# barathanaslan/whisper-ipa

Measured on AMD Instinct MI355X. Metric: audio-seconds/sec transcribed (whisper-small, 30s clips), higher is better.
Workload: dtype bf16

## Files before the change

### include/wipa.h

```cpp
#ifndef WIPA_H
#define WIPA_H
#include <stddef.h>
#include <stdint.h>
#ifdef __cplusplus
extern "C" {
#endif

typedef void* wipa_stream_t;

enum { WIPA_F32 = 0, WIPA_BF16 = 1, WIPA_FP8_E4M3 = 2  };
enum { WIPA_OK = 0, WIPA_ERR_ARG = -1, WIPA_ERR_HIP = -2, WIPA_ERR_STATE = -3 };

#define WIPA_N_SAMPLES 480000
#define WIPA_N_FRAMES 3000
#define WIPA_N_FFT 400
#define WIPA_HOP 160
#define WIPA_HEAD_DIM 64

int wipa_version(void);
const char* wipa_last_error(void);

int wipa_stream_create(wipa_stream_t* out);
int wipa_stream_create_cu_limited(int n_cus, wipa_stream_t* out);
int wipa_stream_destroy(wipa_stream_t s);
// ... 86 lines not shown
int wipa_embed_tokens(const int32_t* tokens, int64_t ld_tok, int B, int T, int t_start, const int32_t* pos_dev,
                      const void* tok_emb, int emb_dtype, const float* emb_scale, const float* pos_emb, float* x, int D,
                      wipa_stream_t s);

typedef struct wipa_attn_desc {
    const void* q;
    const void* k;
    const void* v;
    void* out;
    const int32_t* tk_dev;
    const int32_t* q_row_dev;
    float* lse;
    int64_t q_bs, q_rs, q_hs;
    int64_t k_bs, k_rs, k_hs;
    int64_t v_bs, v_rs, v_hs;
    int64_t o_bs, o_rs, o_hs;
    int32_t B, H, Tq, Tk;
    int32_t causal, dtype;
} wipa_attn_desc;
int wipa_attention(const wipa_attn_desc* d, wipa_stream_t s);

int wipa_flash_attn_enc_bf16(const void* qk, int64_t ldqk, const void* vt, int64_t ldvt, void* out, int64_t ldo,
                             int B, int H, int T, wipa_stream_t s);
int wipa_flash_attn_enc_f32(const float* q, int64_t ldq, const float* k, int64_t ldk, const float* v, int64_t ldv, float* out,
                            int64_t ldo, int B, int H, int T, int f32_split, wipa_stream_t s);

int wipa_decode_attn(const wipa_attn_desc* d, wipa_stream_t s);
int wipa_decode_cross_attn(const void* q, const void* kv, void* out, int B, int H, int Tk, int dtype,
                           wipa_stream_t s);
int wipa_decode_cross_attn_multi(const void* q, const void* kv, void* out, int B, int H, int Tk, int n_q, int dtype,
                                 wipa_stream_t s);

typedef struct wipa_self_block_desc {
    const float* x;
    const float* ln_w;
    const float* ln_b;
    const void* wqkv;
    const float* bqkv;
    const void* wo;
    void* kcache;
    void* vcache;
    const int32_t* pos;
    float* slabs;
    int64_t kv_batch_stride, slab_stride;
    int32_t B, d, H, dtype;
    float eps, qk_scale;
// ... 68 lines not shown
typedef struct wipa_model_cfg {
    int32_t n_mels, n_audio_ctx, n_audio_state, n_audio_head, n_audio_layer;
    int32_t n_vocab, n_text_ctx, n_text_state, n_text_head, n_text_layer;
    int32_t dtype;
    int32_t f32_split;
    int32_t dec_w_dtype;
    int32_t weights_generation;
    int32_t enc_act_fp8;
    int32_t dec_cross_absorbed;
    int32_t dec_cross_splits;
} wipa_model_cfg;

#define WIPA_ENC_GLOBAL 7
#define WIPA_ENC_PER_LAYER 14
#define WIPA_ENC_FP8_PER_LAYER 8
#define WIPA_DEC_GLOBAL 4
#define WIPA_DEC_PER_LAYER 20
#define WIPA_DEC_FP8_PER_LAYER 6
#define WIPA_DEC_ABSORBED_PER_LAYER 1

size_t wipa_encoder_workspace_bytes(const wipa_model_cfg* cfg, int B);
int wipa_encoder_forward(const wipa_model_cfg* cfg, const void* const* weights, const void* mel_padded, void* out,
                         void* workspace, size_t workspace_bytes, int B, wipa_stream_t s);

#define WIPA_PROFILE_CLASSES 4
int wipa_profile_begin(wipa_stream_t s);
int wipa_profile_end(float* ms_by_class, int* launches_by_class);

typedef struct wipa_dec_layout {
    int64_t total_bytes;
    int64_t tokens;
    int64_t ld_tok;
    int64_t pos;
    int64_t not_done;
    int64_t sum_logprobs;
    int64_t logits;
    int64_t ld_logits;
    int64_t cross_kv;
    int64_t self_kv;
    int64_t scratch;
} wipa_dec_layout;
int wipa_decoder_layout(const wipa_model_cfg* cfg, int B, wipa_dec_layout* out);
int wipa_decoder_set_audio(const wipa_model_cfg* cfg, const void* const* weights, const void* features, void* state,
                           size_t state_bytes, int B, wipa_stream_t s);
int wipa_decoder_begin(const wipa_model_cfg* cfg, void* state, size_t state_bytes, int B, const int32_t* initial_tokens_host,
                       int n_init, wipa_stream_t s);
// ... 42 lines not shown
```

### whisper_ipa_amd/_lib.py

```python
from __future__ import annotations

import ctypes as C
import os
import threading

_HERE = os.path.dirname(os.path.abspath(__file__))
LIB_PATH = os.path.join(_HERE, "libwipa.so")

WIPA_F32, WIPA_BF16, WIPA_FP8_E4M3 = 0, 1, 2
GREEDY_PARTS = 2048
RESAMPLE_TILE = 512
ENC_GLOBAL, ENC_PER_LAYER = 7, 14
DEC_GLOBAL, DEC_PER_LAYER, DEC_FP8_PER_LAYER = 4, 20, 6
GEMM_DISPATCH = ("tile128", "tile256", "tile384", "tile384n", "tile256p", "skinny", "skinny_fp8", "skinny_ln", "kmajor", "split_k",
                 "tile_fp8", "tile_fp8_384")
ENC_FP8_PER_LAYER = 8
DEC_ABSORBED_PER_LAYER = 1

c_void_p, c_int, c_int64, c_size_t, c_float = C.c_void_p, C.c_int, C.c_int64, C.c_size_t, C.c_float


class GemmDesc(C.Structure):
    _fields_ = [
        ("A", c_void_p), ("W", c_void_p), ("C", c_void_p), ("bias", c_void_p), ("residual", c_void_p),
# ... 72 lines not shown
    "wipa_stream_create_cu_limited": (c_int, [c_int, C.POINTER(c_void_p)]),
    "wipa_stream_destroy": (c_int, [c_void_p]),
    "wipa_resample_pad": (c_int, [c_void_p, c_size_t, c_void_p, _P(PcmClipDesc), c_int, c_void_p, c_size_t, c_void_p, c_void_p]),
    "wipa_logmel_tables_bytes": (c_size_t, [c_int]),
    "wipa_logmel_init": (c_int, [c_void_p, c_int, c_void_p]),
    "wipa_logmel_workspace_bytes": (c_size_t, [c_int, c_int]),
    "wipa_logmel": (c_int, [c_void_p, c_int, c_int, c_void_p, c_void_p, c_int, c_void_p, c_size_t, c_void_p]),
    "wipa_mel_pad_cast": (c_int, [c_void_p, c_int, c_int, c_void_p, c_int, c_void_p]),
    "wipa_gemm": (c_int, [_P(GemmDesc), c_void_p]),
    "wipa_gemm_dispatch_counts": (c_int, [_P(c_int64), c_int, c_int]),
    "wipa_layernorm": (c_int, [c_void_p, c_int, c_int64, c_void_p, c_int, c_int64, c_void_p, c_void_p, c_int, c_int,
                               c_float, c_void_p]),
    "wipa_layernorm_fp8": (c_int, [c_void_p, c_int64, c_void_p, c_int64, c_void_p, c_void_p, c_void_p, c_int, c_int, c_float, c_void_p]),
    "wipa_rowquant_fp8": (c_int, [c_void_p, c_int, c_int64, c_void_p, c_int64, c_void_p, c_int, c_int, c_void_p]),
    "wipa_add_slabs_layernorm": (c_int, [c_void_p, c_int64, c_void_p, c_int, c_int64, c_void_p, c_int, c_int64, c_void_p,
                                         c_void_p, c_int, c_int, c_float, c_void_p]),
    "wipa_embed_tokens": (c_int, [c_void_p, c_int64, c_int, c_int, c_int, c_void_p, c_void_p, c_int, c_void_p, c_void_p, c_void_p,
                                  c_int, c_void_p]),
    "wipa_attention": (c_int, [_P(AttnDesc), c_void_p]),
    "wipa_flash_attn_enc_f32": (c_int, [c_void_p, c_int64, c_void_p, c_int64, c_void_p, c_int64, c_void_p, c_int64, c_int, c_int,
                                       c_int, c_int, c_void_p]),
    "wipa_flash_attn_enc_bf16": (c_int, [c_void_p, c_int64, c_void_p, c_int64, c_void_p, c_int64, c_int, c_int, c_int,
                                         c_void_p]),
    "wipa_decode_attn": (c_int, [_P(AttnDesc), c_void_p]),
    "wipa_decode_cross_attn": (c_int, [c_void_p, c_void_p, c_void_p, c_int, c_int, c_int, c_int, c_void_p]),
    "wipa_decode_self_block": (c_int, [_P(SelfBlockDesc), c_void_p]),
    "wipa_decode_cross_block": (c_int, [_P(CrossBlockDesc), c_void_p]),
    "wipa_cross_absorbed_splits": (c_int, [c_int, c_int]),
    "wipa_cross_absorbed_resident_groups_for": (c_int, [c_int, c_int, c_int, c_int, c_int64]),
    "wipa_cross_absorbed_resident_groups": (c_int, [c_int, c_int, c_int, c_int]),
    "wipa_cross_absorbed_scratch_bytes": (c_size_t, [c_int, c_int, c_int]),
    "wipa_cross_absorbed_init": (c_int, [c_int]),
    "wipa_cross_absorbed_attention": (c_int, [c_void_p, c_int64, c_void_p, c_void_p, c_void_p, c_void_p, c_void_p, c_int64, c_void_p, c_size_t,
                                              c_int, c_int, c_int, c_int, c_float, c_int, c_void_p]),
    "wipa_cross_absorbed_stream": (c_int, [c_void_p, c_void_p, c_size_t, c_int, c_int, c_int, c_int, c_int, c_void_p]),
    "wipa_decode_cross_absorbed_block": (c_int, [_P(CrossBlockDesc), c_void_p, c_void_p, c_void_p, c_void_p, c_size_t, c_void_p]),
    "wipa_decode_cross_absorbed_block_out": (c_int, [_P(CrossBlockDesc), c_void_p, c_void_p, c_void_p, c_void_p, c_void_p, c_void_p, c_int64,
                                                     c_void_p, c_size_t, c_void_p]),
    "wipa_greedy_step": (c_int, [c_void_p, c_int64, c_int, c_int, c_void_p, c_void_p, c_void_p, c_int64, c_void_p, c_int,
                                 c_int, c_void_p, c_void_p, c_void_p]),
    "wipa_add_i32": (c_int, [c_void_p, C.c_int32, c_void_p]),
    "wipa_greedy_step_embed": (c_int, [c_void_p, c_int64, c_int, c_int, c_void_p, c_void_p, c_void_p, c_int64, c_void_p, c_void_p, c_void_p,
                                       c_int, c_int, c_void_p, c_void_p, c_void_p, c_int, c_void_p, c_void_p, c_int, c_void_p, c_void_p,
                                       c_void_p, c_void_p, c_int, c_int, c_float, c_void_p]),
    "wipa_logits_greedy_supported": (c_int, [c_int, c_int, c_int, c_int]),
    "wipa_logits_greedy_partials_bytes": (c_size_t, [c_int]),
    "wipa_logits_greedy": (c_int, [c_void_p, c_int64, c_void_p, c_int64, c_void_p, c_int64, c_int, c_int, c_int, c_void_p, c_void_p, c_void_p,
                                   c_int, c_void_p, c_size_t, c_void_p]),
    "wipa_greedy_step_embed_partials": (c_int, [c_void_p, c_int, c_int, c_void_p, c_int64, c_void_p, c_void_p, c_void_p, c_int, c_int, c_void_p,
                                                c_void_p, c_void_p, c_int, c_void_p, c_void_p, c_int, c_void_p, c_void_p, c_void_p, c_void_p,
                                                c_int, c_int, c_float, c_void_p]),
    "wipa_embed_layernorm": (c_int, [c_void_p, c_int64, c_int, c_void_p, c_void_p, c_int, c_void_p, c_void_p, c_int, c_void_p, c_void_p,
                                     c_void_p, c_void_p, c_int, c_int, c_float, c_void_p]),
    "wipa_bpe_create": (c_void_p, [c_void_p, c_void_p, c_void_p, c_int]),
    "wipa_bpe_free": (None, [c_void_p]),
    "wipa_bpe_encode_piece": (c_int, [c_void_p, C.c_char_p, c_int, c_void_p, c_int]),
    "wipa_bpe_decode": (c_int, [c_void_p, c_void_p, c_int, c_void_p, c_int]),
    "wipa_build_token_batch": (c_int, [c_void_p, c_void_p, c_int, c_void_p, c_int, C.c_int32, c_void_p, c_int64]),
    "wipa_profile_begin": (c_int, [c_void_p]),
    "wipa_profile_end": (c_int, [_P(c_float), _P(c_int)]),
    "wipa_encoder_workspace_bytes": (c_size_t, [_P(ModelCfg), c_int]),
    "wipa_encoder_forward": (c_int, [_P(ModelCfg), _P(c_void_p), c_void_p, c_void_p, c_void_p, c_size_t, c_int, c_void_p]),
    "wipa_decoder_layout": (c_int, [_P(ModelCfg), c_int, _P(DecLayout)]),
    "wipa_decoder_set_audio": (c_int, [_P(ModelCfg), _P(c_void_p), c_void_p, c_void_p, c_size_t, c_int, c_void_p]),
    "wipa_decoder_begin": (c_int, [_P(ModelCfg), c_void_p, c_size_t, c_int, _P(C.c_int32), c_int, c_void_p]),
    "wipa_decoder_run": (c_int, [_P(ModelCfg), _P(c_void_p), c_void_p, c_size_t, c_int, c_int, c_int, c_void_p, c_void_p, c_int,
                                 c_int, c_void_p]),
    "wipa_decoder_prefill": (c_int, [_P(ModelCfg), _P(c_void_p), c_void_p, c_size_t, c_int, c_int, c_int, c_void_p, c_void_p, c_int,
                                     c_void_p]),
    "wipa_decode_cross_attn_multi": (c_int, [c_void_p, c_void_p, c_void_p, c_int, c_int, c_int, c_int, c_int, c_void_p]),
    "wipa_decoder_release": (c_int, [c_void_p]),
    "wipa_decoder_logits_workspace_bytes": (c_size_t, [_P(ModelCfg), c_int, c_int]),
    "wipa_decoder_logits": (c_int, [_P(ModelCfg), _P(c_void_p), c_void_p, c_void_p, c_void_p, c_int64, c_void_p, c_size_t,
                                    c_int, c_int, c_void_p]),
    "wipa_masked_ce": (c_int, [c_void_p, c_int64, c_void_p, c_int64, c_int, c_int, c_int, c_int, c_void_p, c_void_p,
                               c_void_p]),
    "wipa_transpose": (c_int, [c_void_p, c_int64, c_void_p, c_int64, c_int, c_int, c_int, c_int, c_void_p]),
    "wipa_sum_slabs": (c_int, [c_void_p, c_int, c_int64, c_void_p, c_int64, c_int, c_void_p]),
    "wipa_sum_slabs_ex": (c_int, [c_void_p, c_int, c_int64, c_void_p, c_int64, c_void_p, c_float, c_void_p]),
    "wipa_colsum": (c_int, [c_void_p, c_int64, c_int, c_int, c_void_p, c_int, c_void_p, c_int64, c_void_p]),
    "wipa_layernorm_bwd": (c_int, [c_void_p, c_void_p, c_void_p, c_void_p, c_int, c_void_p, c_void_p, c_void_p, c_int64, c_int, c_int,
                                   c_float, c_void_p]),
    "wipa_gelu": (c_int, [c_void_p, c_void_p, c_int64, c_void_p]),
    "wipa_gelu_bwd": (c_int, [c_void_p, c_void_p, c_void_p, c_int64, c_void_p]),
    "wipa_masked_ce_bwd": (c_int, [c_void_p, c_int64, c_void_p, c_int64, c_int, c_int, c_int, c_void_p, c_void_p, c_void_p]),
# ... 40 lines not shown
```

### whisper_ipa_amd/csrc/attention.hip

```cpp
#include <cstring>

#include "attn_stream.h"
#include "wipa_common.h"

namespace {

struct AttnParams {
    const char* q;
    const char* k;
    const char* v;
    char* out;
    const int32_t* tk_dev;
    const int32_t* q_row_dev;
    float* lse;
    int64_t q_bs, q_rs, q_hs, k_bs, k_rs, k_hs, v_bs, v_rs, v_hs, o_bs, o_rs, o_hs;
    int Tq, Tk, causal, H;
};

constexpr int GA_LD = 68;

template <typename T>
__global__ __launch_bounds__(256) void attn_generic_kernel(AttnParams p) {
    __shared__ __attribute__((aligned(16))) float Ks[64 * GA_LD];
    __shared__ __attribute__((aligned(16))) float Vs[64 * GA_LD];
// ... 343 lines not shown
        const f32x2 l2e = {LOG2E, LOG2E}, mneg = {-m_new, -m_new};                                 \
        _Pragma("unroll") for (int u = 0; u < 2; ++u)                                              \
            _Pragma("unroll") for (int i = 0; i < 16; i += 2) {                                    \
                const f32x2 x = __builtin_elementwise_fma(f32x2{S[u][i], S[u][i + 1]}, l2e, mneg); \
                const f32x2 pv = {__builtin_amdgcn_exp2f(x.x), __builtin_amdgcn_exp2f(x.y)};       \
                S[u][i] = pv.x;                                                                    \
                S[u][i + 1] = pv.y;                                                                \
                psum2 += pv;                                                                       \
            }                                                                                      \
        const float psum = psum2.x + psum2.y;                                                      \
        if (__any(m_new > m)) {                                                                    \
            const float alpha = __builtin_amdgcn_exp2f(m - m_new);                                 \
            l *= alpha;                                                                            \
            _Pragma("unroll") for (int i = 0; i < 16; ++i) {                                       \
                O[0][i] *= alpha;                                                                  \
                O[1][i] *= alpha;                                                                  \
            }                                                                                      \
            m = m_new;                                                                             \
        }                                                                                          \
        l += psum;                                                                                 \
    } while (0)
#define WIPA_FLASH_SOFTMAX_FINISH() l += __shfl_xor(l, 32, 64)

__global__ __launch_bounds__(512) void flash_enc_bf16_kernel(const __bf16* __restrict__ qk, int64_t ldqk,
                                                             const __bf16* __restrict__ vt, int64_t ldvt,
                                                             __bf16* __restrict__ out, int64_t ldo, int H, int T) {
    __shared__ __attribute__((aligned(16))) char smem[4 * FA_TILE];
    const int tid = threadIdx.x, lane = tid & 63, wave = tid >> 6;
    const int r = lane & 31, hh = lane >> 5;
    const int h = blockIdx.y, b = blockIdx.z;
    const int D = H * 64;
    const int nw = blockDim.x >> 6;
    const int q0 = blockIdx.x * (nw * 32) + wave * 32;
    const int nkt = (T + 63) / 64;

    bf16x8 qf[4];
    {
        const int qrow = min(q0 + r, T - 1);
        const __bf16* qp = qk + ((int64_t)b * T + qrow) * ldqk + h * 64 + 8 * hh;
#pragma unroll
        for (int s = 0; s < 4; ++s) qf[s] = *reinterpret_cast<const bf16x8*>(qp + 16 * s);
    }
    typedef __attribute__((address_space(3))) void* lds_t;
    const __bf16* kbase = qk + (int64_t)b * T * ldqk + D + h * 64;
    const __bf16* vbase = vt + ((int64_t)b * D + h * 64) * ldvt;
    const __amdgpu_buffer_rsrc_t rK = __builtin_amdgcn_make_buffer_rsrc((void*)kbase, 0, (int)(((int64_t)(T - 1) * ldqk + 64) * 2), 0x00020000);
    const __amdgpu_buffer_rsrc_t rV = __builtin_amdgcn_make_buffer_rsrc((void*)vbase, 0, (int)(((int64_t)63 * ldvt + ldvt) * 2), 0x00020000);
    const int wv = __builtin_amdgcn_readfirstlane(wave);
    const int ppw = 8 / nw;
    int offK[2], offV[2];
#pragma unroll
    for (int i = 0; i < 2; ++i) {
        const int row = 8 * (ppw * wv + i) + (lane >> 3);
        const int c = (lane & 7) ^ ((row >> 1) & 7);
        offK[i] = row * (int)ldqk * 2 + c * 16;
        offV[i] = row * (int)ldvt * 2 + c * 16;
    }
    auto stage = [&](int kt, int buf) {
        char* base = smem + buf * 2 * FA_TILE + (ppw * wv) * 1024;
        const int k0 = kt * 64;
#pragma unroll
        for (int i = 0; i < 2; ++i) {
            if (i < ppw) {
                __builtin_amdgcn_raw_ptr_buffer_load_lds(rK, (lds_t)(base + i * 1024), 16, offK[i], k0 * (int)ldqk * 2, 0, 0);
                __builtin_amdgcn_raw_ptr_buffer_load_lds(rV, (lds_t)(base + FA_TILE + i * 1024), 16, offV[i], k0 * 2, 0, 0);
            }
        }
    };

    f32x16 O[2];
#pragma unroll
    for (int i = 0; i < 16; ++i) O[0][i] = O[1][i] = 0.f;
    float m = NEG_BIG, l = 0.f;
    const int rsw = (r >> 1) & 7;

    stage(0, 0);
    asm volatile("s_waitcnt vmcnt(0)" ::: "memory");
    __syncthreads();
    for (int kt = 0; kt < nkt; ++kt) {
        if (kt + 1 < nkt) stage(kt + 1, (kt + 1) & 1);
        const char* kbuf = smem + (kt & 1) * 2 * FA_TILE;
        const char* vbuf = kbuf + FA_TILE;
        f32x16 S[2];
#pragma unroll
        for (int u = 0; u < 2; ++u) {
#pragma unroll
            for (int i = 0; i < 16; ++i) S[u][i] = 0.f;
            const char* krow = kbuf + (32 * u + r) * FA_ROWB;
#pragma unroll
            for (int s = 0; s < 4; ++s) {
                const bf16x8 kf = *reinterpret_cast<const bf16x8*>(krow + (((2 * s + hh) ^ rsw) << 4));
                S[u] = __builtin_amdgcn_mfma_f32_32x32x16_bf16(kf, qf[s], S[u], 0, 0, 0);
            }
        }
        WIPA_FLASH_SOFTMAX_TILE();
#pragma unroll
        for (int u = 0; u < 2; ++u)
#pragma unroll
            for (int sp = 0; sp < 2; ++sp) {
                bf16x8 pb;
#pragma unroll
                for (int j = 0; j < 8; ++j) pb[j] = (__bf16)S[u][8 * sp + j];
#pragma unroll
                for (int dt = 0; dt < 2; ++dt) {
                    const char* vrow = vbuf + (32 * dt + r) * FA_ROWB + 8 * hh;
                    const int c0 = 4 * u + 2 * sp;
                    const bf16x4 lo = *reinterpret_cast<const bf16x4*>(vrow + ((c0 ^ rsw) << 4));
                    const bf16x4 hi = *reinterpret_cast<const bf16x4*>(vrow + (((c0 + 1) ^ rsw) << 4));
                    const bf16x8 vf = {lo[0], lo[1], lo[2], lo[3], hi[0], hi[1], hi[2], hi[3]};
                    O[dt] = __builtin_amdgcn_mfma_f32_32x32x16_bf16(vf, pb, O[dt], 0, 0, 0);
                    asm volatile("" ::: "memory");
                }
            }
        asm volatile("s_waitcnt vmcnt(0)" ::: "memory");
        __syncthreads();
    }
// ... 172 lines not shown
                             f32x4{S[u][8 * sp + 4], S[u][8 * sp + 5], S[u][8 * sp + 6], S[u][8 * sp + 7]}, ph, pl);
#pragma unroll
                for (int dt = 0; dt < 2; ++dt) {
                    const float* vr = vbuf + (32 * dt + r) * FF_LD + 32 * u + 16 * sp + 4 * hh;
                    bf16x8 vh, vl;
                    split_bf16x2(*reinterpret_cast<const f32x4*>(vr), *reinterpret_cast<const f32x4*>(vr + 8), vh, vl);
                    O[dt] = __builtin_amdgcn_mfma_f32_32x32x16_bf16(vh, pl, O[dt], 0, 0, 0);
                    O[dt] = __builtin_amdgcn_mfma_f32_32x32x16_bf16(vl, ph, O[dt], 0, 0, 0);
                    O[dt] = __builtin_amdgcn_mfma_f32_32x32x16_bf16(vh, ph, O[dt], 0, 0, 0);
                }
            }
        WIPA_FLASH_F32_TILE_END();
    }
    WIPA_FLASH_F32_TAIL();
}

#undef WIPA_FLASH_F32_INDICES
#undef WIPA_FLASH_F32_STAGING
#undef WIPA_FLASH_F32_TILE_BEGIN
#undef WIPA_FLASH_F32_TILE_END
#undef WIPA_FLASH_F32_TAIL
#undef WIPA_FLASH_SOFTMAX_TILE
#undef WIPA_FLASH_SOFTMAX_FINISH

}

static bool attn_strides_aligned(const wipa_attn_desc* d) {
    const int64_t al = d->dtype == WIPA_BF16 ? 8 : 4;
    return d->q_rs % al == 0 && d->k_rs % al == 0 && d->v_rs % al == 0 && d->q_hs % al == 0 && d->k_hs % al == 0 && d->v_hs % al == 0 &&
           d->q_bs % al == 0 && d->k_bs % al == 0 && d->v_bs % al == 0;
}

static void fill_attn_params(const wipa_attn_desc* d, AttnParams& p) {
    p.q = (const char*)d->q;
    p.k = (const char*)d->k;
    p.v = (const char*)d->v;
    p.out = (char*)d->out;
    p.tk_dev = d->tk_dev;
    p.q_row_dev = d->q_row_dev;
    p.lse = d->lse;
    p.q_bs = d->q_bs; p.q_rs = d->q_rs; p.q_hs = d->q_hs;
    p.k_bs = d->k_bs; p.k_rs = d->k_rs; p.k_hs = d->k_hs;
    p.v_bs = d->v_bs; p.v_rs = d->v_rs; p.v_hs = d->v_hs;
    p.o_bs = d->o_bs; p.o_rs = d->o_rs; p.o_hs = d->o_hs;
    p.Tq = d->Tq;
    p.Tk = d->Tk;
// ... 13 lines not shown
    if (d->dtype == WIPA_F32 && !valu && d->Tq >= 16 && !d->tk_dev && !d->q_row_dev && d->o_rs % 4 == 0 && d->o_hs % 4 == 0 &&
        d->o_bs % 4 == 0) {
        hipLaunchKernelGGL(attn_fwd_f32_mfma_kernel, dim3((d->Tq + 63) / 64, d->H, d->B), dim3(256), 0, (hipStream_t)stream, p);
        WIPA_LAUNCH_CHECK();
        return WIPA_OK;
    }
    if (d->dtype == WIPA_F32)
        hipLaunchKernelGGL((attn_generic_kernel<float>), grid, dim3(256), 0, (hipStream_t)stream, p);
    else
        hipLaunchKernelGGL((attn_generic_kernel<__bf16>), grid, dim3(256), 0, (hipStream_t)stream, p);
    WIPA_LAUNCH_CHECK();
    return WIPA_OK;
}

extern "C" int wipa_flash_attn_enc_bf16(const void* qk, int64_t ldqk, const void* vt, int64_t ldvt, void* out, int64_t ldo,
                                        int B, int H, int T, wipa_stream_t stream) {
    WIPA_REQUIRE(qk && vt && out, "wipa_flash_attn_enc_bf16: null pointer");
    WIPA_REQUIRE(ldqk % 8 == 0 && ldvt % 8 == 0 && ldo % 4 == 0, "wipa_flash_attn_enc_bf16: ld alignment");
    WIPA_REQUIRE(ldvt >= ((T + 63) / 64) * 64, "wipa_flash_attn_enc_bf16: ldvt=%lld must cover ceil64(T)", (long long)ldvt);
    WIPA_REQUIRE(B > 0 && H > 0 && T > 0, "wipa_flash_attn_enc_bf16: bad shape");
    static const int q128 = [] { const char* e = getenv("WIPA_FLASH_Q128"); return e ? atoi(e) : 0; }();
    const int nw = (T > 256 && !q128) ? 8 : 4;
    dim3 grid((T + nw * 32 - 1) / (nw * 32), H, B);
    hipLaunchKernelGGL(flash_enc_bf16_kernel, grid, dim3(nw * 64), 0, (hipStream_t)stream, (const __bf16*)qk, ldqk,
                       (const __bf16*)vt, ldvt, (__bf16*)out, ldo, H, T);
    WIPA_LAUNCH_CHECK();
    return WIPA_OK;
}

extern "C" int wipa_flash_attn_enc_f32(const float* q, int64_t ldq, const float* k, int64_t ldk, const float* v, int64_t ldv,
                                       float* out, int64_t ldo, int B, int H, int T, int f32_split, wipa_stream_t stream) {
    WIPA_REQUIRE(q && k && v && out, "wipa_flash_attn_enc_f32: null pointer");
    WIPA_REQUIRE(ldq % 4 == 0 && ldk % 4 == 0 && ldv % 4 == 0 && ldo % 4 == 0, "wipa_flash_attn_enc_f32: row strides must be multiples of 4");
    WIPA_REQUIRE(((uintptr_t)q % 16) == 0 && ((uintptr_t)k % 16) == 0 && ((uintptr_t)v % 16) == 0 && ((uintptr_t)out % 16) == 0,
                 "wipa_flash_attn_enc_f32: operands must be 16-byte aligned");
    WIPA_REQUIRE(B > 0 && H > 0 && T > 0, "wipa_flash_attn_enc_f32: bad shape");
    dim3 grid((T + 127) / 128, H, B);
    if (!f32_split)
        hipLaunchKernelGGL(flash_enc_f32_kernel, grid, dim3(256), 0, (hipStream_t)stream, q, ldq, k, ldk, v, ldv, out, ldo, T);
    else
        hipLaunchKernelGGL(flash_enc_f32s_kernel, grid, dim3(256), 0, (hipStream_t)stream, q, ldq, k, ldk, v, ldv, out, ldo, T);
    WIPA_LAUNCH_CHECK();
    return WIPA_OK;
}

extern "C" int wipa_decode_attn(const wipa_attn_desc* d, wipa_stream_t stream) {
    WIPA_REQUIRE(d && d->q && d->k && d->v && d->out, "wipa_decode_attn: null pointer");
    WIPA_REQUIRE(d->B > 0 && d->H > 0 && d->Tq == 1, "wipa_decode_attn: one query row per (b,h) (Tq=%d)", d->Tq);
// ... 74 lines not shown
```

### whisper_ipa_amd/csrc/runtime.hip

```cpp
#include <algorithm>
#include <cstdarg>
#include <cstdlib>
#include <cstring>
#include <strings.h>
#include <map>
#include <mutex>
#include <tuple>
#include <vector>

#include "wipa_common.h"

static thread_local char g_err[512] = "";
void wipa_set_error(const char* fmt, ...) {
    va_list ap;
    va_start(ap, fmt);
    vsnprintf(g_err, sizeof(g_err), fmt, ap);
    va_end(ap);
}
extern "C" const char* wipa_last_error(void) { return g_err; }
extern "C" int wipa_version(void) { return 100; }

extern "C" int wipa_stream_create_cu_limited(int n_cus, wipa_stream_t* out) {
    int dev = 0, total = 0;
    WIPA_CHECK_HIP(hipGetDevice(&dev));
// ... 142 lines not shown
    g.bias = bias; g.act = act; g.residual = residual;
    g.a_scale = a_scale; g.w_scale = w_scale;
    return wipa_gemm(&g, s);
}

struct EncWs {
    size_t c1, x, ln, qk, v, ao, h, total;
};
EncWs enc_ws(const wipa_model_cfg* c, int B) {
    const size_t e = wipa_dtype_size(c->dtype), d = c->n_audio_state, M = (size_t)B * c->n_audio_ctx;
    EncWs w;
    size_t o = 0;
    w.c1 = o; o += align256(((size_t)B * ROWS_IN + 4) * d * e);
    w.x = o;  o += align256(M * d * 4);
    w.ln = o; o += align256(M * d * e);
    w.qk = o; o += align256(M * 2 * d * e);
    w.v = o;  o += align256(c->dtype == WIPA_BF16 ? (size_t)B * d * T_ENC_PAD * e + 256 : M * d * e);
    w.ao = o; o += align256(M * d * e);
    w.h = o;  o += align256(M * 4 * d * e);
    w.total = o;
    return w;
}

}

extern "C" size_t wipa_encoder_workspace_bytes(const wipa_model_cfg* cfg, int B) {
    if (!cfg || B <= 0) return 0;
    return enc_ws(cfg, B).total;
}

extern "C" int wipa_encoder_forward(const wipa_model_cfg* cfg, const void* const* w, const void* mel_padded, void* out,
                                    void* workspace, size_t workspace_bytes, int B, wipa_stream_t stream) {
    RT_CALL(cfg_check(cfg));
    SplitScope split_scope(cfg);
    WIPA_REQUIRE(w && mel_padded && out && workspace && B > 0, "wipa_encoder_forward: null pointer / bad batch");
    const EncWs L = enc_ws(cfg, B);
    WIPA_REQUIRE(workspace_bytes >= L.total, "wipa_encoder_forward: workspace too small (%zu < %zu)", workspace_bytes, L.total);
    hipStream_t s = (hipStream_t)stream;
    const int dt = cfg->dtype;
    const size_t e = wipa_dtype_size(dt);
    const int d = cfg->n_audio_state, H = cfg->n_audio_head, T = cfg->n_audio_ctx, M = B * T;
    char* ws = (char*)workspace;
    void* c1 = ws + L.c1;
    float* x = (float*)(ws + L.x);
    void* ln = ws + L.ln;
    void* qk = ws + L.qk;
    void* vb = ws + L.v;
    void* ao = ws + L.ao;
    void* hb = ws + L.h;
    const int K1 = round_up(3 * cfg->n_mels, k_multiple(dt));

    WIPA_CHECK_HIP(hipMemsetAsync(c1, 0, (size_t)d * e, s));
    {
        wipa_gemm_desc g;
        memset(&g, 0, sizeof(g));
        g.rg_in = ROWS_IN; g.rg_valid = WIPA_N_FRAMES; g.rg_stride = (int64_t)ROWS_IN * d; g.zero_invalid_rows = 1;
        g.c_offset = d;
        PROF(PROF_GEMM, gemm(mel_padded, cfg->n_mels, w[0], K1, c1, d, B * ROWS_IN, d, K1, dt, dt, (const float*)w[1], 1, nullptr,
                     stream, &g));
    }
    {
        wipa_gemm_desc g;
        memset(&g, 0, sizeof(g));
        g.rg_in = T + 1; g.rg_valid = T; g.rg_stride = (int64_t)T * d;
        g.pos = (const float*)w[4]; g.ldpos = d;
        PROF(PROF_GEMM, gemm(c1, 2 * d, w[2], 3 * d, x, d, B * (T + 1), d, 3 * d, dt, WIPA_F32, (const float*)w[3], 1, nullptr,
                     stream, &g));
    }
    if (dt == WIPA_BF16) WIPA_CHECK_HIP(hipMemsetAsync(vb, 0, (size_t)B * d * T_ENC_PAD * e, s));
    const bool f8 = cfg->enc_act_fp8 != 0;
    float* ln_scale = (float*)((char*)ln + (size_t)M * d);
    const void* const* w8 = w + WIPA_ENC_GLOBAL + WIPA_ENC_PER_LAYER * cfg->n_audio_layer;
    for (int l = 0; l < cfg->n_audio_layer; ++l) {
        const void* const* lw = w + WIPA_ENC_GLOBAL + WIPA_ENC_PER_LAYER * l;
        const void* const* l8 = w8 + WIPA_ENC_FP8_PER_LAYER * l;
        if (f8) PROF(PROF_NORM, wipa_layernorm_fp8(x, d, ln, d, ln_scale, (const float*)lw[0], (const float*)lw[1], M, d, 1e-5f, stream));
        else PROF(PROF_NORM, wipa_layernorm(x, WIPA_F32, d, ln, dt, d, (const float*)lw[0], (const float*)lw[1], M, d, 1e-5f, stream));
        {
            wipa_gemm_desc g;
            memset(&g, 0, sizeof(g));
            g.col_scale_n = 2 * d; g.col_scale = QK_SCALE;
            if (f8) PROF(PROF_GEMM, gemm_f8(ln, d, ln_scale, l8[0], d, (const float*)l8[1], qk, 2 * d, M, 2 * d, d, dt, (const float*)lw[3], 0,
                                            nullptr, stream, &g));
            else PROF(PROF_GEMM, gemm(ln, d, lw[2], d, qk, 2 * d, M, 2 * d, d, dt, dt, (const float*)lw[3], 0, nullptr, stream, &g));
        }
        if (dt == WIPA_BF16) {
            wipa_gemm_desc g;
            memset(&g, 0, sizeof(g));
            g.bias_along_m = 1; g.cg_in = T; g.cg_stride = (int64_t)d * T_ENC_PAD;
            if (f8) PROF(PROF_GEMM, gemm_f8(l8[2], d, (const float*)l8[3], ln, d, ln_scale, vb, T_ENC_PAD, d, M, d, dt, (const float*)lw[5], 0,
                                            nullptr, stream, &g));
            else PROF(PROF_GEMM, gemm(lw[4], d, ln, d, vb, T_ENC_PAD, d, M, d, dt, dt, (const float*)lw[5], 0, nullptr, stream, &g));
            PROF(PROF_ATTN, wipa_flash_attn_enc_bf16(qk, 2 * d, vb, T_ENC_PAD, ao, d, B, H, T, stream));
        } else {
            PROF(PROF_GEMM, gemm(ln, d, lw[4], d, vb, d, M, d, d, dt, dt, (const float*)lw[5], 0, nullptr, stream));
            PROF(PROF_ATTN, wipa_flash_attn_enc_f32((const float*)qk, 2 * d, (const float*)qk + d, 2 * d, (const float*)vb, d, (float*)ao, d,
                                            B, H, T, t_f32_split, stream));
        }
        PROF(PROF_GEMM, gemm(ao, d, lw[6], d, x, d, M, d, d, dt, WIPA_F32, (const float*)lw[7], 0, x, stream));
        if (f8) {
            PROF(PROF_NORM, wipa_layernorm_fp8(x, d, ln, d, ln_scale, (const float*)lw[8], (const float*)lw[9], M, d, 1e-5f, stream));
            PROF(PROF_GEMM, gemm_f8(ln, d, ln_scale, l8[4], d, (const float*)l8[5], hb, 4 * d, M, 4 * d, d, dt, (const float*)lw[11], 1, nullptr,
                                    stream));
            void* h8 = qk;
            float* h_scale = (float*)ao;
            PROF(PROF_NORM, wipa_rowquant_fp8(hb, dt, 4 * d, h8, 4 * d, h_scale, M, 4 * d, stream));
            PROF(PROF_GEMM, gemm_f8(h8, 4 * d, h_scale, l8[6], 4 * d, (const float*)l8[7], x, d, M, d, 4 * d, WIPA_F32, (const float*)lw[13], 0,
                                    x, stream));
        } else {
// ... 802 lines not shown
```

### whisper_ipa_amd/ops.py

```python
from __future__ import annotations

import ctypes as C
from typing import Optional

import torch

from . import _lib
from .runtime import dt_code, on_stream, ptr, sptr


def gemm(A: torch.Tensor, W: torch.Tensor, C_out: torch.Tensor, *, M: int, N: int, K: int, lda: int, ldw: int, ldc: int,
         bias: Optional[torch.Tensor] = None, bias_along_m: bool = False, act: int = 0,
         residual: Optional[torch.Tensor] = None, pos: Optional[torch.Tensor] = None, ldpos: int = 0,
         col_scale_n: int = 0, col_scale: float = 1.0, rg_in: int = 0, rg_valid: int = 0, rg_stride: int = 0,
         cg_in: int = 0, cg_stride: int = 0, c_offset: int = 0, c_offset_dev: Optional[torch.Tensor] = None,
         zero_invalid_rows: bool = False, k_slices: int = 0, slab_stride: int = 0, f32_split: bool = False,
         a_trans: bool = False, w_trans: bool = False) -> torch.Tensor:
    L = _lib.lib()
    d = _lib.GemmDesc()
    d.A, d.W, d.C = ptr(A), ptr(W), ptr(C_out)
    d.bias, d.residual, d.pos, d.c_offset_dev = ptr(bias), ptr(residual), ptr(pos), ptr(c_offset_dev)
    d.lda, d.ldw, d.ldc, d.ldpos = lda, ldw, ldc, ldpos
    d.rg_stride, d.cg_stride, d.c_offset = rg_stride, cg_stride, c_offset
    d.M, d.N, d.K = M, N, K
# ... 115 lines not shown
        out = torch.empty(B, H, 64, dtype=q.dtype, device=q.device)
        d = _lib.AttnDesc()
        d.q, d.k, d.v, d.out = ptr(q), ptr(k), ptr(v), ptr(out)
        d.tk_dev, d.q_row_dev = ptr(tk_dev), ptr(q_row_dev)
        d.q_bs, d.q_rs, d.q_hs = q.stride(0), q.stride(1), q.stride(2)
        d.k_bs, d.k_rs, d.k_hs = k.stride(0), k.stride(1), k.stride(2)
        d.v_bs, d.v_rs, d.v_hs = v.stride(0), v.stride(1), v.stride(2)
        d.o_bs, d.o_rs, d.o_hs = out.stride(0), out.stride(0), out.stride(1)
        d.B, d.H, d.Tq, d.Tk, d.causal, d.dtype = B, H, 1, (k.shape[1] if Tk is None else Tk), 0, dt_code(q.dtype)
        _lib.check(L.wipa_decode_attn(C.byref(d), sptr(s)), "wipa_decode_attn")
    return out


def flash_attn_enc(qk: torch.Tensor, vt: torch.Tensor, B: int, H: int, T: int) -> torch.Tensor:
    L = _lib.lib()
    D = H * 64
    with on_stream() as s:
        out = torch.empty(B * T, D, dtype=torch.bfloat16, device=qk.device)
        _lib.check(L.wipa_flash_attn_enc_bf16(ptr(qk), qk.stride(0), ptr(vt), vt.stride(1), ptr(out), D, B, H, T, sptr(s)),
                   "wipa_flash_attn_enc_bf16")
    return out


def flash_attn_enc_f32(qk: torch.Tensor, v: torch.Tensor, B: int, H: int, T: int, f32_split: bool = False) -> torch.Tensor:
    L = _lib.lib()
    D = H * 64
    assert qk.dtype == torch.float32 and v.dtype == torch.float32
    with on_stream() as s:
        out = torch.empty(B * T, D, dtype=torch.float32, device=qk.device)
        k = qk[:, D:]
        _lib.check(L.wipa_flash_attn_enc_f32(ptr(qk), qk.stride(0), ptr(k), qk.stride(0), ptr(v), v.stride(0), ptr(out), D,
                                             B, H, T, int(f32_split), sptr(s)), "wipa_flash_attn_enc_f32")
    return out


def decode_cross_attn(q: torch.Tensor, kv: torch.Tensor) -> torch.Tensor:
    L = _lib.lib()
    B, twoH, Tk, hd = kv.shape
    assert hd == 64 and kv.is_contiguous() and q.is_contiguous()
    with on_stream() as s:
        out = torch.empty_like(q)
        _lib.check(L.wipa_decode_cross_attn(ptr(q), ptr(kv), ptr(out), B, twoH // 2, Tk, dt_code(q.dtype), sptr(s)),
                   "wipa_decode_cross_attn")
    return out


# ... 22 lines not shown
```

### whisper_ipa_amd/whisper.py

```python
from __future__ import annotations

import ctypes as C
import math
from dataclasses import dataclass, asdict
from typing import Dict, List, Optional

import torch

from . import _lib
from .audio import N_FRAMES, PADDED_FRAMES, padded_mel_rows
from .runtime import device, dt_code, on_stream, ptr, ptr_table, sptr, stream, stream_id


@dataclass
class ModelDimensions:
    n_mels: int
    n_audio_ctx: int
    n_audio_state: int
    n_audio_head: int
    n_audio_layer: int
    n_vocab: int
    n_text_ctx: int
    n_text_state: int
    n_text_head: int
# ... 144 lines not shown
        if strict and missing:
            raise KeyError(f"missing weights: {missing[:5]} ... ({len(missing)})")
        with on_stream():
            for n in names:
                if n in flat:
                    t = torch.as_tensor(flat[n]).detach()
                    want = self.dtype if _is_matrix(n, t) else torch.float32
                    self._params[n] = t.to(device=self.device, dtype=want).contiguous()
                    if n.startswith("encoder."):
                        self._enc_generation += 1
        self._fp8 = {}
        self._fp8_enc = {}
        self._invalidate()
        return self

    @property
    def weights_format(self) -> str:
        return "fp8_e4m3" if self._fp8 else str(self.dtype).replace("torch.", "")

    @property
    def activations_format(self) -> str:
        return "fp8_e4m3" if self._fp8_enc else str(self.dtype).replace("torch.", "")

    def quantize_weights(self, fmt: str = "fp8_e4m3", activations: str = "bf16"):
        if fmt != "fp8_e4m3":
            raise _lib.WipaError(f"quantize_weights: unknown format {fmt!r} (fp8_e4m3)")
        if self.dtype != torch.bfloat16:
            raise _lib.WipaError("quantize_weights: fp8 weights run with bf16 activations: call set_dtype(torch.bfloat16) first")
        if activations not in ("bf16", "fp8"):
            raise _lib.WipaError(f"quantize_weights: activations must be 'bf16' or 'fp8', got {activations!r}")
        if activations == "fp8" and self.dims.n_audio_state % 128 != 0:
            raise _lib.WipaError("quantize_weights: fp8 activations need an encoder width that is a multiple of 128")
        step = set(_decode_step_matrices(self.dims))
        enc_f8 = set()
        if activations == "fp8":
            for i in range(self.dims.n_audio_layer):
                pfx = f"encoder.blocks.{i}"
                enc_f8 |= {f"{pfx}.attn.query.weight", f"{pfx}.attn.key.weight", f"{pfx}.attn.value.weight", f"{pfx}.mlp1.weight",
                           f"{pfx}.mlp2.weight"}
        fp8, fp8_enc = {}, {}
        with on_stream():
            for n, t in list(self._params.items()):
                if not _is_matrix(n, t):
                    continue
                codes, scale = quantize_fp8_e4m3(t)
                self._params[n] = dequantize_fp8_e4m3(codes, scale).to(torch.bfloat16).reshape(t.shape).contiguous()
# ... 103 lines not shown
        return self._packed_abs

    def _pack(self, fp8: bool):
        P, T, d = self._params, self.dtype, self.dims
        kmul = 64 if T == torch.bfloat16 else 32
        f32 = torch.float32
        with on_stream():
            def mat(x):
                return x.to(T).contiguous()

            def vec(x):
                return x.to(f32).contiguous()

            de = d.n_audio_state
            K1 = (3 * d.n_mels + kmul - 1) // kmul * kmul
            c1 = torch.zeros(de, K1, dtype=T, device=self.device)
            c1[:, : 3 * d.n_mels] = P["encoder.conv1.weight"].reshape(de, 3 * d.n_mels).to(T)
            enc = [c1, vec(P["encoder.conv1.bias"]), mat(P["encoder.conv2.weight"].reshape(de, 3 * de)),
                   vec(P["encoder.conv2.bias"]), vec(self._enc_pos), vec(P["encoder.ln_post.weight"]),
                   vec(P["encoder.ln_post.bias"])]
            for i in range(d.n_audio_layer):
                p = f"encoder.blocks.{i}"
                qb = P[f"{p}.attn.query.bias"]
                enc += [vec(P[f"{p}.attn_ln.weight"]), vec(P[f"{p}.attn_ln.bias"]),
                        mat(torch.cat([P[f"{p}.attn.query.weight"], P[f"{p}.attn.key.weight"]], 0)),
                        vec(torch.cat([qb.float(), torch.zeros_like(qb, dtype=f32)], 0)),
                        mat(P[f"{p}.attn.value.weight"]), vec(P[f"{p}.attn.value.bias"]),
                        mat(P[f"{p}.attn.out.weight"]), vec(P[f"{p}.attn.out.bias"]),
                        vec(P[f"{p}.mlp_ln.weight"]), vec(P[f"{p}.mlp_ln.bias"]),
                        mat(P[f"{p}.mlp1.weight"]), vec(P[f"{p}.mlp1.bias"]),
                        mat(P[f"{p}.mlp2.weight"]), vec(P[f"{p}.mlp2.bias"])]
            dec = [mat(P["decoder.token_embedding.weight"]), vec(P["decoder.positional_embedding"]),
                   vec(P["decoder.ln.weight"]), vec(P["decoder.ln.bias"])]
            for i in range(d.n_text_layer):
                p = f"decoder.blocks.{i}"
                qb, vb = P[f"{p}.attn.query.bias"].float(), P[f"{p}.attn.value.bias"].float()
                cvb = P[f"{p}.cross_attn.value.bias"].float()
                z = torch.zeros_like(qb)
                dec += [vec(P[f"{p}.attn_ln.weight"]), vec(P[f"{p}.attn_ln.bias"]),
                        mat(torch.cat([P[f"{p}.attn.query.weight"], P[f"{p}.attn.key.weight"], P[f"{p}.attn.value.weight"]], 0)),
                        vec(torch.cat([qb, z, vb], 0)),
                        mat(P[f"{p}.attn.out.weight"]), vec(P[f"{p}.attn.out.bias"]),
                        vec(P[f"{p}.cross_attn_ln.weight"]), vec(P[f"{p}.cross_attn_ln.bias"]),
                        mat(P[f"{p}.cross_attn.query.weight"]), vec(P[f"{p}.cross_attn.query.bias"]),
                        mat(torch.cat([P[f"{p}.cross_attn.key.weight"], P[f"{p}.cross_attn.value.weight"]], 0)),
                        vec(torch.cat([z, cvb], 0)),
                        mat(P[f"{p}.cross_attn.out.weight"]), vec(P[f"{p}.cross_attn.out.bias"]),
                        vec(P[f"{p}.mlp_ln.weight"]), vec(P[f"{p}.mlp_ln.bias"]),
                        mat(P[f"{p}.mlp1.weight"]), vec(P[f"{p}.mlp1.bias"]),
                        mat(P[f"{p}.mlp2.weight"]), vec(P[f"{p}.mlp2.bias"])]
# ... 129 lines not shown
```

Before: 26840.

## Fuse encoder Q/K/V projection and read row-major V in flash attention

Packs encoder query, key and value weights contiguously so a single GEMM writes a row-major q|k|v buffer, replacing the separate transposed V GEMM and its zeroing memset. A new flash-attention variant reads V row-major and uses ds_read_b64_tr_b16 LDS transpose loads to form the MFMA operands. This removes one GEMM launch and the memset per layer, at the cost of a new LDS swizzle and transpose path that has to be correct.

New measurement: 26960 (median of 6 runs). About the same (+0.5%).

```diff
diff --git a/include/wipa.h b/include/wipa.h
--- a/include/wipa.h
+++ b/include/wipa.h
@@ -132,6 +132,7 @@
 
 int wipa_flash_attn_enc_bf16(const void* qk, int64_t ldqk, const void* vt, int64_t ldvt, void* out, int64_t ldo,
                              int B, int H, int T, wipa_stream_t s);
+int wipa_flash_attn_enc_bf16_rm(const void* qkv, int64_t ldqkv, void* out, int64_t ldo, int B, int H, int T, wipa_stream_t s);
 int wipa_flash_attn_enc_f32(const float* q, int64_t ldq, const float* k, int64_t ldk, const float* v, int64_t ldv, float* out,
                             int64_t ldo, int B, int H, int T, int f32_split, wipa_stream_t s);
 
@@ -246,6 +247,7 @@
 size_t wipa_encoder_workspace_bytes(const wipa_model_cfg* cfg, int B);
 int wipa_encoder_forward(const wipa_model_cfg* cfg, const void* const* weights, const void* mel_padded, void* out,
                          void* workspace, size_t workspace_bytes, int B, wipa_stream_t s);
+int wipa_encoder_qkv_fused(const wipa_model_cfg* cfg, const void* const* weights);
 
 #define WIPA_PROFILE_CLASSES 4
 int wipa_profile_begin(wipa_stream_t s);
diff --git a/whisper_ipa_amd/_lib.py b/whisper_ipa_amd/_lib.py
--- a/whisper_ipa_amd/_lib.py
+++ b/whisper_ipa_amd/_lib.py
@@ -118,6 +118,7 @@
                                        c_int, c_int, c_void_p]),
     "wipa_flash_attn_enc_bf16": (c_int, [c_void_p, c_int64, c_void_p, c_int64, c_void_p, c_int64, c_int, c_int, c_int,
                                          c_void_p]),
+    "wipa_flash_attn_enc_bf16_rm": (c_int, [c_void_p, c_int64, c_void_p, c_int64, c_int, c_int, c_int, c_void_p]),
     "wipa_decode_attn": (c_int, [_P(AttnDesc), c_void_p]),
     "wipa_decode_cross_attn": (c_int, [c_void_p, c_void_p, c_void_p, c_int, c_int, c_int, c_int, c_void_p]),
     "wipa_decode_self_block": (c_int, [_P(SelfBlockDesc), c_void_p]),
@@ -157,6 +158,7 @@
     "wipa_profile_end": (c_int, [_P(c_float), _P(c_int)]),
     "wipa_encoder_workspace_bytes": (c_size_t, [_P(ModelCfg), c_int]),
     "wipa_encoder_forward": (c_int, [_P(ModelCfg), _P(c_void_p), c_void_p, c_void_p, c_void_p, c_size_t, c_int, c_void_p]),
+    "wipa_encoder_qkv_fused": (c_int, [_P(ModelCfg), _P(c_void_p)]),
     "wipa_decoder_layout": (c_int, [_P(ModelCfg), c_int, _P(DecLayout)]),
     "wipa_decoder_set_audio": (c_int, [_P(ModelCfg), _P(c_void_p), c_void_p, c_void_p, c_size_t, c_int, c_void_p]),
     "wipa_decoder_begin": (c_int, [_P(ModelCfg), c_void_p, c_size_t, c_int, _P(C.c_int32), c_int, c_void_p]),
diff --git a/whisper_ipa_amd/csrc/attention.hip b/whisper_ipa_amd/csrc/attention.hip
--- a/whisper_ipa_amd/csrc/attention.hip
+++ b/whisper_ipa_amd/csrc/attention.hip
@@ -389,6 +389,17 @@
     } while (0)
 #define WIPA_FLASH_SOFTMAX_FINISH() l += __shfl_xor(l, 32, 64)
 
+typedef int fa_v2i32 __attribute__((ext_vector_type(2)));
+typedef int fa_v4i32 __attribute__((ext_vector_type(4)));
+#define WIPA_FLASH_TR4(X, A0, A1, LO, HI)                                                                            \
+    asm volatile("ds_read_b64_tr_b16 %0, %4 offset:" #LO "\n\tds_read_b64_tr_b16 %1, %4 offset:" #HI                 \
+                 "\n\tds_read_b64_tr_b16 %2, %5 offset:" #LO "\n\tds_read_b64_tr_b16 %3, %5 offset:" #HI             \
+                 "\n\ts_waitcnt lgkmcnt(0)"                                                                          \
+                 : "=&v"(X[0]), "=&v"(X[1]), "=&v"(X[2]), "=&v"(X[3])                                                \
+                 : "v"(A0), "v"(A1)                                                                                  \
+                 : "memory")
+
+template <bool VRM>
 __global__ __launch_bounds__(512) void flash_enc_bf16_kernel(const __bf16* __restrict__ qk, int64_t ldqk,
                                                              const __bf16* __restrict__ vt, int64_t ldvt,
                                                              __bf16* __restrict__ out, int64_t ldo, int H, int T) {
@@ -410,9 +421,10 @@
     }
     typedef __attribute__((address_space(3))) void* lds_t;
     const __bf16* kbase = qk + (int64_t)b * T * ldqk + D + h * 64;
-    const __bf16* vbase = vt + ((int64_t)b * D + h * 64) * ldvt;
+    const __bf16* vbase = VRM ? vt + (int64_t)b * T * ldvt + h * 64 : vt + ((int64_t)b * D + h * 64) * ldvt;
     const __amdgpu_buffer_rsrc_t rK = __builtin_amdgcn_make_buffer_rsrc((void*)kbase, 0, (int)(((int64_t)(T - 1) * ldqk + 64) * 2), 0x00020000);
-    const __amdgpu_buffer_rsrc_t rV = __builtin_amdgcn_make_buffer_rsrc((void*)vbase, 0, (int)(((int64_t)63 * ldvt + ldvt) * 2), 0x00020000);
+    const __amdgpu_buffer_rsrc_t rV = __builtin_amdgcn_make_buffer_rsrc(
+        (void*)vbase, 0, VRM ? (int)(((int64_t)(T - 1) * ldvt + 64) * 2) : (int)(((int64_t)63 * ldvt + ldvt) * 2), 0x00020000);
     const int wv = __builtin_amdgcn_readfirstlane(wave);
     const int ppw = 8 / nw;
     int offK[2], offV[2];
@@ -421,7 +433,8 @@
         const int row = 8 * (ppw * wv + i) + (lane >> 3);
         const int c = (lane & 7) ^ ((row >> 1) & 7);
         offK[i] = row * (int)ldqk * 2 + c * 16;
-        offV[i] = row * (int)ldvt * 2 + c * 16;
+        if constexpr (VRM) offV[i] = row * (int)ldvt * 2 + ((lane & 7) ^ ((row & 2) << 1)) * 16;
+        else offV[i] = row * (int)ldvt * 2 + c * 16;
     }
     auto stage = [&](int kt, int buf) {
         char* base = smem + buf * 2 * FA_TILE + (ppw * wv) * 1024;
@@ -430,7 +443,8 @@
         for (int i = 0; i < 2; ++i) {
             if (i < ppw) {
                 __builtin_amdgcn_raw_ptr_buffer_load_lds(rK, (lds_t)(base + i * 1024), 16, offK[i], k0 * (int)ldqk * 2, 0, 0);
-                __builtin_amdgcn_raw_ptr_buffer_load_lds(rV, (lds_t)(base + FA_TILE + i * 1024), 16, offV[i], k0 * 2, 0, 0);
+                __builtin_amdgcn_raw_ptr_buffer_load_lds(rV, (lds_t)(base + FA_TILE + i * 1024), 16, offV[i],
+                                                         VRM ? k0 * (int)ldvt * 2 : k0 * 2, 0, 0);
             }
         }
     };
@@ -440,6 +454,14 @@
     for (int i = 0; i < 16; ++i) O[0][i] = O[1][i] = 0.f;
     float m = NEG_BIG, l = 0.f;
     const int rsw = (r >> 1) & 7;
+    unsigned vtr[2] = {0u, 0u};
+    if constexpr (VRM) {
+        const int q = (lane >> 2) & 3, p = lane & 3, gl = (lane >> 4) & 1;
+#pragma unroll
+        for (int dt = 0; dt < 2; ++dt)
+            vtr[dt] = (unsigned)(uintptr_t)(lds_t)smem + FA_TILE + (4 * hh + q) * FA_ROWB +
+                      (((4 * dt + 2 * gl + (p >> 1)) ^ ((q & 2) << 1)) << 4) + 8 * (p & 1);
+    }
 
     stage(0, 0);
     asm volatile("s_waitcnt vmcnt(0)" ::: "memory");
@@ -459,6 +481,29 @@
                 const bf16x8 kf = *reinterpret_cast<const bf16x8*>(krow + (((2 * s + hh) ^ rsw) << 4));
                 S[u] = __builtin_amdgcn_mfma_f32_32x32x16_bf16(kf, qf[s], S[u], 0, 0, 0);
             }
+        }
+        if constexpr (VRM) {
+            const unsigned a0 = vtr[0] + (kt & 1) * 2 * FA_TILE, a1 = vtr[1] + (kt & 1) * 2 * FA_TILE;
+            fa_v2i32 va[2][4];
+            WIPA_FLASH_TR4(va[0], a0, a1, 0, 1024);
+            WIPA_FLASH_SOFTMAX_TILE();
+#pragma unroll
+            for (int st = 0; st < 4; ++st) {
+                bf16x8 pb;
+#pragma unroll
+                for (int j = 0; j < 8; ++j) pb[j] = (__bf16)S[st >> 1][8 * (st & 1) + j];
+                const fa_v2i32* x = va[st & 1];
+                O[0] = __builtin_amdgcn_mfma_f32_32x32x16_bf16(__builtin_bit_cast(bf16x8, fa_v4i32{x[0][0], x[0][1], x[1][0], x[1][1]}),
+                                                               pb, O[0], 0, 0, 0);
+                O[1] = __builtin_amdgcn_mfma_f32_32x32x16_bf16(__builtin_bit_cast(bf16x8, fa_v4i32{x[2][0], x[2][1], x[3][0], x[3][1]}),
+                                                               pb, O[1], 0, 0, 0);
+                if (st == 0) WIPA_FLASH_TR4(va[1], a0, a1, 2048, 3072);
+                if (st == 1) WIPA_FLASH_TR4(va[0], a0, a1, 4096, 5120);
+                if (st == 2) WIPA_FLASH_TR4(va[1], a0, a1, 6144, 7168);
+            }
+            asm volatile("s_waitcnt vmcnt(0)" ::: "memory");
+            __syncthreads();
+            continue;
         }
         WIPA_FLASH_SOFTMAX_TILE();
 #pragma unroll
@@ -677,6 +722,7 @@
 #undef WIPA_FLASH_F32_TAIL
 #undef WIPA_FLASH_SOFTMAX_TILE
 #undef WIPA_FLASH_SOFTMAX_FINISH
+#undef WIPA_FLASH_TR4
 
 }
 
@@ -736,8 +782,25 @@
     static const int q128 = [] { const char* e = getenv("WIPA_FLASH_Q128"); return e ? atoi(e) : 0; }();
     const int nw = (T > 256 && !q128) ? 8 : 4;
     dim3 grid((T + nw * 32 - 1) / (nw * 32), H, B);
-    hipLaunchKernelGGL(flash_enc_bf16_kernel, grid, dim3(nw * 64), 0, (hipStream_t)stream, (const __bf16*)qk, ldqk,
+    hipLaunchKernelGGL(flash_enc_bf16_kernel<false>, grid, dim3(nw * 64), 0, (hipStream_t)stream, (const __bf16*)qk, ldqk,
                        (const __bf16*)vt, ldvt, (__bf16*)out, ldo, H, T);
+    WIPA_LAUNCH_CHECK();
+    return WIPA_OK;
+}
+
+extern "C" int wipa_flash_attn_enc_bf16_rm(const void* qkv, int64_t ldqkv, void* out, int64_t ldo, int B, int H, int T,
+                                           wipa_stream_t stream) {
+    WIPA_REQUIRE(qkv && out, "wipa_flash_attn_enc_bf16_rm: null pointer");
+    WIPA_REQUIRE(B > 0 && H > 0 && T > 0, "wipa_flash_attn_enc_bf16_rm: bad shape");
+    WIPA_REQUIRE(ldqkv % 8 == 0 && ldo % 4 == 0 && ldqkv >= 3 * 64 * (int64_t)H, "wipa_flash_attn_enc_bf16_rm: ld alignment");
+    WIPA_REQUIRE(((uintptr_t)qkv % 16) == 0, "wipa_flash_attn_enc_bf16_rm: qkv must be 16-byte aligned");
+    WIPA_REQUIRE((int64_t)T * ldqkv * 2 < (int64_t)1 << 31, "wipa_flash_attn_enc_bf16_rm: a clip's rows must span less than 2 GiB");
+    static const int q128 = [] { const char* e = getenv("WIPA_FLASH_Q128"); return e ? atoi(e) : 0; }();
+    const int nw = (T > 256 && !q128) ? 8 : 4;
+    dim3 grid((T + nw * 32 - 1) / (nw * 32), H, B);
+    const __bf16* p = (const __bf16*)qkv;
+    hipLaunchKernelGGL(flash_enc_bf16_kernel<true>, grid, dim3(nw * 64), 0, (hipStream_t)stream, p, ldqkv, p + 2 * 64 * (int64_t)H, ldqkv,
+                       (__bf16*)out, ldo, H, T);
     WIPA_LAUNCH_CHECK();
     return WIPA_OK;
 }
diff --git a/whisper_ipa_amd/csrc/runtime.hip b/whisper_ipa_amd/csrc/runtime.hip
--- a/whisper_ipa_amd/csrc/runtime.hip
+++ b/whisper_ipa_amd/csrc/runtime.hip
@@ -188,6 +188,23 @@
     return w;
 }
 
+bool enc_qkv_fused(const wipa_model_cfg* c, const void* const* w) {
+    if (c->dtype != WIPA_BF16 || c->enc_act_fp8) return false;
+    const char* env = getenv("WIPA_ENC_QKV_FUSED");
+    if (env && !strcmp(env, "0")) return false;
+    const size_t d = c->n_audio_state;
+    if ((size_t)c->n_audio_ctx * 3 * d * 2 >= ((size_t)1 << 31)) return false;
+    for (int l = 0; l < c->n_audio_layer; ++l) {
+        const void* const* lw = w + WIPA_ENC_GLOBAL + WIPA_ENC_PER_LAYER * l;
+        if ((const char*)lw[4] != (const char*)lw[2] + 2 * d * d * 2 || (const float*)lw[5] != (const float*)lw[3] + 2 * d) return false;
+    }
+    return true;
+}
+
+}
+
+extern "C" int wipa_encoder_qkv_fused(const wipa_model_cfg* cfg, const void* const* w) {
+    return cfg && w && cfg_check(cfg) == WIPA_OK && enc_qkv_fused(cfg, w) ? 1 : 0;
 }
 
 extern "C" size_t wipa_encoder_workspace_bytes(const wipa_model_cfg* cfg, int B) {
@@ -233,7 +250,9 @@
         PROF(PROF_GEMM, gemm(c1, 2 * d, w[2], 3 * d, x, d, B * (T + 1), d, 3 * d, dt, WIPA_F32, (const float*)w[3], 1, nullptr,
                      stream, &g));
     }
-    if (dt == WIPA_BF16) WIPA_CHECK_HIP(hipMemsetAsync(vb, 0, (size_t)B * d * T_ENC_PAD * e, s));
+    const bool fused = enc_qkv_fused(cfg, w);
+    WIPA_REQUIRE(!fused || L.qk + (size_t)M * 3 * d * e <= L.ao, "wipa_encoder_forward: q|k|v does not fit the q|k and v regions");
+    if (dt == WIPA_BF16 && !fused) WIPA_CHECK_HIP(hipMemsetAsync(vb, 0, (size_t)B * d * T_ENC_PAD * e, s));
     const bool f8 = cfg->enc_act_fp8 != 0;
     float* ln_scale = (float*)((char*)ln + (size_t)M * d);
     const void* const* w8 = w + WIPA_ENC_GLOBAL + WIPA_ENC_PER_LAYER * cfg->n_audio_layer;
@@ -246,11 +265,14 @@
             wipa_gemm_desc g;
             memset(&g, 0, sizeof(g));
             g.col_scale_n = 2 * d; g.col_scale = QK_SCALE;
+            const int nq = fused ? 3 * d : 2 * d;
             if (f8) PROF(PROF_GEMM, gemm_f8(ln, d, ln_scale, l8[0], d, (const float*)l8[1], qk, 2 * d, M, 2 * d, d, dt, (const float*)lw[3], 0,
                                             nullptr, stream, &g));
-            else PROF(PROF_GEMM, gemm(ln, d, lw[2], d, qk, 2 * d, M, 2 * d, d, dt, dt, (const float*)lw[3], 0, nullptr, stream, &g));
-        }
-        if (dt == WIPA_BF16) {
+            else PROF(PROF_GEMM, gemm(ln, d, lw[2], d, qk, nq, M, nq, d, dt, dt, (const float*)lw[3], 0, nullptr, stream, &g));
+        }
+        if (fused) {
+            PROF(PROF_ATTN, wipa_flash_attn_enc_bf16_rm(qk, 3 * d, ao, d, B, H, T, stream));
+        } else if (dt == WIPA_BF16) {
             wipa_gemm_desc g;
             memset(&g, 0, sizeof(g));
             g.bias_along_m = 1; g.cg_in = T; g.cg_stride = (int64_t)d * T_ENC_PAD;
diff --git a/whisper_ipa_amd/ops.py b/whisper_ipa_amd/ops.py
--- a/whisper_ipa_amd/ops.py
+++ b/whisper_ipa_amd/ops.py
@@ -161,6 +161,15 @@
     return out
 
 
+def flash_attn_enc_rm(qkv: torch.Tensor, B: int, H: int, T: int) -> torch.Tensor:
+    L = _lib.lib()
+    D = H * 64
+    with on_stream() as s:
+        out = torch.empty(B * T, D, dtype=torch.bfloat16, device=qkv.device)
+        _lib.check(L.wipa_flash_attn_enc_bf16_rm(ptr(qkv), qkv.stride(0), ptr(out), D, B, H, T, sptr(s)), "wipa_flash_attn_enc_bf16_rm")
+    return out
+
+
 def flash_attn_enc_f32(qk: torch.Tensor, v: torch.Tensor, B: int, H: int, T: int, f32_split: bool = False) -> torch.Tensor:
     L = _lib.lib()
     D = H * 64
diff --git a/whisper_ipa_amd/whisper.py b/whisper_ipa_amd/whisper.py
--- a/whisper_ipa_amd/whisper.py
+++ b/whisper_ipa_amd/whisper.py
@@ -190,6 +190,11 @@
     def activations_format(self) -> str:
         return "fp8_e4m3" if self._fp8_enc else str(self.dtype).replace("torch.", "")
 
+    @property
+    def encoder_qkv_fused(self) -> bool:
+        pk = self.packed()
+        return bool(_lib.lib().wipa_encoder_qkv_fused(C.byref(pk["cfg"]), pk["enc_tab"]))
+
     def quantize_weights(self, fmt: str = "fp8_e4m3", activations: str = "bf16"):
         if fmt != "fp8_e4m3":
             raise _lib.WipaError(f"quantize_weights: unknown format {fmt!r} (fp8_e4m3)")
@@ -339,10 +344,10 @@
             for i in range(d.n_audio_layer):
                 p = f"encoder.blocks.{i}"
                 qb = P[f"{p}.attn.query.bias"]
+                wqkv = mat(torch.cat([P[f"{p}.attn.query.weight"], P[f"{p}.attn.key.weight"], P[f"{p}.attn.value.weight"]], 0))
+                bqkv = vec(torch.cat([qb.float(), torch.zeros_like(qb, dtype=f32), P[f"{p}.attn.value.bias"].float()], 0))
                 enc += [vec(P[f"{p}.attn_ln.weight"]), vec(P[f"{p}.attn_ln.bias"]),
-                        mat(torch.cat([P[f"{p}.attn.query.weight"], P[f"{p}.attn.key.weight"]], 0)),
-                        vec(torch.cat([qb.float(), torch.zeros_like(qb, dtype=f32)], 0)),
-                        mat(P[f"{p}.attn.value.weight"]), vec(P[f"{p}.attn.value.bias"]),
+                        wqkv[: 2 * de], bqkv[: 2 * de], wqkv[2 * de:], bqkv[2 * de:],
                         mat(P[f"{p}.attn.out.weight"]), vec(P[f"{p}.attn.out.bias"]),
                         vec(P[f"{p}.mlp_ln.weight"]), vec(P[f"{p}.mlp_ln.bias"]),
                         mat(P[f"{p}.mlp1.weight"]), vec(P[f"{p}.mlp1.bias"]),
```
